# cloudflare/circl

Measured on AMD Instinct MI355X. Metric: ML-KEM-768 encapsulations/sec (whole node), batch=2^20, higher is better.
Workload: dtype i32; 1 GPU; ML-KEM-768 Encapsulate, distinct-key (one GPU-generated key per item), batch=1048576 per GPU, inputs resident in HBM (SURVEY 8d scope i; the PCIe-inclusive host-ABI rate, scope ii, is `value_host_abi`); key_pool=1048576, parallelism=batch split per device, no collectives, mode=encaps

## Files before the change

### circl_amd/csrc/api_mlkem.hip

```cpp
#include "host_common.h"
#include "keytable.h"
#include "mlkem_kernels.h"

using namespace circl::host;
using circl::KeyIdx;

namespace {

constexpr size_t kKemWsPerItem = 129;
size_t kem_scratch_bytes() { return 256 + max_resident_blocks() * 64 * 512; }
size_t kem_small_batch() {
    static const size_t v = [] {
        const char *e = getenv("CIRCL_HIP_KEM_SMALL");
        const int lg = e ? atoi(e) : 15;
        return lg <= 0 ? size_t(0) : size_t(1) << std::min(lg, 20);
    }();
    return v;
}
size_t kem_coop_batch() {
    static const size_t v = [] {
        const char *e = getenv("CIRCL_HIP_KEM_COOP");
        const int lg = e ? atoi(e) : 11;
        return lg <= 0 ? size_t(0) : size_t(1) << std::min(lg, 20);
    }();
// ... 51 lines not shown
struct KemWs {
    uint8_t *slot0, *slot1, *slot2, *slot3, *status_slot;
    unsigned *work;
    uint8_t *scratch;
    KemWs(void *ws, size_t n) {
        slot0 = static_cast<uint8_t *>(ws);
        slot1 = slot0 + 32 * n;
        slot2 = slot0 + 64 * n;
        slot3 = slot0 + 96 * n;
        status_slot = slot0 + 128 * n;
        work = reinterpret_cast<unsigned *>(slot0 + up256(kKemWsPerItem * n));
        scratch = slot0 + up256(kKemWsPerItem * n) + 256;
    }
};


template <int K, bool R3 = false>
int encaps_dev_impl(const uint8_t *ek, const uint8_t *m, uint8_t *ct, uint8_t *ss, uint8_t *status, size_t n,
                    void *ws, size_t ws_bytes, hipStream_t st) {
    using Gm = circl::mlkem::Geom<K>;
    using namespace circl::mlkem;
    if (n == 0) return CIRCL_HIP_OK;
    if (ws_bytes < kem_ws_min(n) || !aligned16(ws) || !aligned16(ek) || !aligned16(m) || !aligned16(ct) || !aligned16(ss))
        return CIRCL_HIP_EWORKSPACE;
    KemWs w(ws, n);
    uint8_t *r_ws = w.slot0, *m_ws = w.slot1;
    const unsigned hb = (unsigned)((n + 255) / 256);
    if (!R3 && n <= kem_chain_item_batch()) {
        ProfScope ps(CIRCL_HIP_KERNEL_MLKEM_ENCRYPT, st);
        hipLaunchKernelGGL((mlkem_encaps_chain_kernel<K, false>), dim3((unsigned)n), dim3(128), 0, st, ek, (size_t)Gm::EK, KeyIdx{},
                           (const int16_t *)nullptr, (const uint8_t *)nullptr, m, ct, ss, status, n);
        HIP_TRY(hipGetLastError());
        return CIRCL_HIP_OK;
    }
    if (!R3 && kem_small_route(n, ws_bytes)) {
        int16_t *key_rows = reinterpret_cast<int16_t *>(static_cast<uint8_t *>(ws) + kem_small_table_ofs(n));
        const int coop = kem_hash_form(n, kem_coop_batch());
        const unsigned nb_expand = (unsigned)((n + Gm::G - 1) / Gm::G), nb_hash = kem_hash_blocks(n, coop);
        static_assert(Gm::LDS_FIFO >= 108 * 8, "the cooperative hash's exchange area fits the FIFO area");
        const size_t want = kem_small_group(n);
        HIP_TRY(hipMemsetAsync(w.work, 0, 256, st));
        {
            ProfScope ps(CIRCL_HIP_KERNEL_MLKEM_HASH, st);
            hipLaunchKernelGGL(mlkem_small_pre_kernel<K>, dim3(nb_hash + nb_expand), dim3(64), Gm::LDS_FIFO, st, ek, m, ss, r_ws, key_rows, n, nb_hash, coop);
        }
        auto kern = mlkem_encrypt_kernel<K, ENCAPS, 0, true, KM_KEYED>;
        const unsigned eb = std::min<unsigned>((unsigned)((n + want - 1) / want), resident_blocks(kern, Gm::LDS_SHARED_TOTAL));
        ProfScope ps(CIRCL_HIP_KERNEL_MLKEM_ENCRYPT, st);
        hipLaunchKernelGGL(kern, dim3(eb), dim3(64), Gm::LDS_SHARED_TOTAL, st, ek, (size_t)Gm::EK, m, (const uint8_t *)r_ws, ct, ss, status,
                           (const uint8_t *)nullptr, (const uint8_t *)nullptr, w.scratch, w.work, n, KeyIdx{}, (const int16_t *)key_rows);
        HIP_TRY(hipGetLastError());
        return CIRCL_HIP_OK;
    }
    HIP_TRY(hipMemsetAsync(w.work, 0, 256, st));
    {
        ProfScope ps(CIRCL_HIP_KERNEL_MLKEM_HASH, st);
        if (R3) hipLaunchKernelGGL(kyber_r3_hash_kernel<K>, dim3(hb), dim3(256), 0, st, ek, m, ss, r_ws, m_ws, n);
        else hipLaunchKernelGGL(mlkem_hash_kernel<K>, dim3(hb), dim3(256), 0, st, ek, m, ss, r_ws, n);
    }
    {
        auto kern = mlkem_encrypt_kernel<K, R3 ? ENCAPS_LENIENT : ENCAPS, 0, true>;
        const unsigned eb = std::min<unsigned>((unsigned)((n + Gm::G - 1) / Gm::G), resident_blocks(kern, Gm::LDS_SCRATCH_TOTAL));
        ProfScope ps(CIRCL_HIP_KERNEL_MLKEM_ENCRYPT, st);
        hipLaunchKernelGGL(kern, dim3(eb), dim3(64), Gm::LDS_SCRATCH_TOTAL, st, ek, (size_t)Gm::EK, R3 ? (const uint8_t *)m_ws : m, (const uint8_t *)r_ws,
                           ct, ss, status, (const uint8_t *)nullptr, (const uint8_t *)nullptr, w.scratch, w.work, n, KeyIdx{},
                           (const int16_t *)nullptr);
    }
    if (R3) {
        ProfScope ps(CIRCL_HIP_KERNEL_MLKEM_HASH, st);
        hipLaunchKernelGGL(kyber_r3_finish_kernel<K>, dim3(hb), dim3(256), 0, st, (const uint8_t *)ct, ss, n);
    }
    HIP_TRY(hipGetLastError());
    return CIRCL_HIP_OK;
}

template <int K>
int encaps_shared_dev_impl(const uint8_t *ek, const uint8_t *m, uint8_t *ct, uint8_t *ss, uint8_t *status, size_t n, void *ws,
                           size_t ws_bytes, hipStream_t st) {
    using Gm = circl::mlkem::Geom<K>;
    using namespace circl::mlkem;
    if (n == 0) return CIRCL_HIP_OK;
    if (ws_bytes < kem_ws_min(n) || !aligned16(ws) || !aligned16(ek) || !aligned16(m) || !aligned16(ct) || !aligned16(ss))
        return CIRCL_HIP_EWORKSPACE;
    KemWs w(ws, n);
    uint8_t *r_ws = w.slot0, *h_ws = w.slot1;
    if (n <= kem_chain_item_batch()) {
        ProfScope ps(CIRCL_HIP_KERNEL_MLKEM_ENCRYPT, st);
        hipLaunchKernelGGL((mlkem_encaps_chain_kernel<K, false>), dim3((unsigned)n), dim3(128), 0, st, ek, (size_t)0, KeyIdx{},
                           (const int16_t *)nullptr, (const uint8_t *)nullptr, m, ct, ss, status, n);
        HIP_TRY(hipGetLastError());
        return CIRCL_HIP_OK;
    }
    HIP_TRY(hipMemsetAsync(w.work, 0, 256, st));
    if (n <= kem_small_shared_batch(false)) {
        int16_t *key_rows = reinterpret_cast<int16_t *>(static_cast<uint8_t *>(ws) + kem_small_table_ofs(n));
        static_assert(Gm::LDS_FIFO >= 108 * 8, "the cooperative hash's exchange area fits the FIFO area");
        {
            ProfScope ps(CIRCL_HIP_KERNEL_MLKEM_HASH, st);
            hipLaunchKernelGGL(mlkem_small_shared_pre_kernel<K>, dim3(1 + (unsigned)((n + 31) / 32)), dim3(64), Gm::LDS_FIFO, st, ek, m, ss, r_ws, key_rows, n);
        }
        auto kern = mlkem_encrypt_kernel<K, ENCAPS, 0, true, KM_KEYED>;
        const size_t want = kem_small_group(n);
        const unsigned eb = std::min<unsigned>((unsigned)((n + want - 1) / want), resident_blocks(kern, Gm::LDS_SHARED_TOTAL));
        ProfScope ps(CIRCL_HIP_KERNEL_MLKEM_ENCRYPT, st);
        hipLaunchKernelGGL(kern, dim3(eb), dim3(64), Gm::LDS_SHARED_TOTAL, st, ek, (size_t)0, m, (const uint8_t *)r_ws, ct, ss, status,
                           (const uint8_t *)nullptr, (const uint8_t *)nullptr, w.scratch, w.work, n, KeyIdx{}, (const int16_t *)key_rows);
        HIP_TRY(hipGetLastError());
        return CIRCL_HIP_OK;
    }
    {
        ProfScope ps(CIRCL_HIP_KERNEL_MLKEM_HASH, st);
        hipLaunchKernelGGL(mlkem_hek_kernel<K>, dim3(1), dim3(64), 0, st, ek, h_ws);
        hipLaunchKernelGGL(mlkem_g_shared_kernel, dim3((unsigned)((n + 255) / 256)), dim3(256), 0, st, (const uint8_t *)h_ws, m, ss,
                           r_ws, n, KeyIdx{});
    }
    {
        auto kern = mlkem_encrypt_kernel<K, ENCAPS, 0, true, KM_SHARED>;
        const unsigned eb = std::min<unsigned>((unsigned)((n + Gm::GS - 1) / Gm::GS), resident_blocks(kern, Gm::LDS_SHARED_TOTAL));
// ... 794 lines not shown
```

### circl_amd/csrc/mlkem_kernels.h

```cpp
#pragma once
#include "kyber_dev.h"

#ifndef CIRCL_KEM_RING_PRIO
#define CIRCL_KEM_RING_PRIO 1
#endif
#ifndef CIRCL_KEM_WAVES_PER_EU
#define CIRCL_KEM_WAVES_PER_EU 4
#endif

namespace circl {
namespace mlkem {

using kyber::Q;

template <int K> struct Params;
template <> struct Params<2> { static constexpr int ETA1 = 3, DU = 10, DV = 4; };
template <> struct Params<3> { static constexpr int ETA1 = 2, DU = 10, DV = 4; };
template <> struct Params<4> { static constexpr int ETA1 = 2, DU = 11, DV = 5; };

template <int K> struct Geom {
    using P = Params<K>;
    static constexpr int EK = 384 * K + 32;
    static constexpr int DK = 768 * K + 96;
    static constexpr int CT = 32 * (P::DU * K + P::DV);
    static constexpr int PAIRS = K * K;
    static constexpr int G = 64 / PAIRS;
    static constexpr int A_STREAMS = G * PAIRS;
    static constexpr int NOISE = 2 * K + 1;
    static constexpr int A_STRIDE = 520;
    static constexpr int NOISE_BYTES = 64 * P::ETA1;
    static constexpr int NOISE_STRIDE = NOISE_BYTES + 8;
    static constexpr int LDS_A = A_STREAMS * A_STRIDE;
    static constexpr int HALVES = K == 2 ? 2 : 1;
    static constexpr int GH = G / HALVES;
    static constexpr int LDS_NOISE = GH * NOISE * NOISE_STRIDE;
    static constexpr int LDS_XCH = 1024;
    static constexpr int LDS_TOTAL = LDS_A + LDS_NOISE + LDS_XCH;
    static constexpr int FIFO_STRIDE = 80;
    static constexpr int LDS_FIFO = 64 * FIFO_STRIDE;
    static constexpr int LDS_SCRATCH_TOTAL = (LDS_FIFO > LDS_NOISE + LDS_XCH) ? LDS_FIFO : LDS_NOISE + LDS_XCH;
    static constexpr int SCRATCH_BYTES = 64 * 512;
    static constexpr int GS = K == 2 ? 8 : 64 / NOISE;
    static constexpr int LDS_NOISE_SHARED = GS * NOISE * NOISE_STRIDE;
    static constexpr int LDS_SHARED_TOTAL = (LDS_FIFO > LDS_NOISE_SHARED + LDS_XCH) ? LDS_FIFO : LDS_NOISE_SHARED + LDS_XCH;
};


template <int FIRST, int COUNT> __device__ __forceinline__ void xor_words(KeccakState &s, const uint64_t *p) {
    detail::static_for<0, COUNT>([&](auto ic) {
        constexpr int i = decltype(ic)::v;
        const uint64_t w = p[i];
        s.lo[FIRST + i] ^= (uint32_t)w;
        s.hi[FIRST + i] ^= (uint32_t)(w >> 32);
    });
}

template <int NWORDS> __device__ __forceinline__ void sha3_256_words(KeccakState &s, const uint64_t *p) {
    constexpr int FULL = NWORDS / 17, REM = NWORDS % 17;
    keccak_zero(s);
#pragma unroll 1
    for (int b = 0; b < FULL; b++) {
        xor_words<0, 17>(s, p + 17 * b);
        keccak_f1600(s);
    }
    xor_words<0, REM>(s, p + 17 * FULL);
    s.lo[REM] ^= kDsSha3;
    s.hi[16] ^= 0x80000000u;
    keccak_f1600(s);
}

__device__ __forceinline__ void sha3_512_m_h(KeccakState &g, const uint64_t *m, const KeccakState &h) {
    keccak_zero(g);
    xor_words<0, 4>(g, m);
#pragma unroll
    for (int i = 0; i < 4; i++) { g.lo[4 + i] = h.lo[i]; g.hi[4 + i] = h.hi[i]; }
    g.lo[8] = kDsSha3;
    g.hi[8] = 0x80000000u;
    keccak_f1600(g);
}

template <int NWORDS, class Src> __device__ __forceinline__ void split_sponge17_src(SplitState &s, Src &&src, uint32_t ds, bool hi_lane) {
    constexpr int FULL = NWORDS / 17, REM = NWORDS % 17;
    uint32_t nx[17];
#pragma unroll
    for (int j = 0; j < 25; j++) s.w[j] = 0;
#pragma unroll
    for (int j = 0; j < 17; j++) nx[j] = (FULL > 0 || j < REM) ? src(j) : 0;
#pragma unroll 1
    for (int b = 0; b < FULL; b++) {
#pragma unroll
        for (int j = 0; j < 17; j++) s.w[j] ^= nx[j];
        const bool last = b + 1 == FULL;
#pragma unroll
// ... 13 lines not shown
                                              size_t item, bool live, int parity) {
    const bool hi_lane = parity != 0;
    const uint32_t *mw = reinterpret_cast<const uint32_t *>(m + item * 32) + parity;
    SplitState s;
#pragma unroll
    for (int j = 0; j < 4; j++) { s.w[j] = mw[2 * j]; s.w[4 + j] = h[j]; }
    s.w[8] = hi_lane ? 0x80000000u : kDsSha3;
#pragma unroll
    for (int j = 9; j < 25; j++) s.w[j] = 0;
    keccak_f1600_split(s, hi_lane);
    if (live) {
        uint32_t *kd = reinterpret_cast<uint32_t *>(ss + item * 32) + parity, *rd = reinterpret_cast<uint32_t *>(r_ws + item * 32) + parity;
#pragma unroll
        for (int j = 0; j < 4; j++) { kd[2 * j] = s.w[j]; rd[2 * j] = s.w[4 + j]; }
    }
}
template <int K>
__device__ __forceinline__ void mlkem_hash_split(const uint8_t *__restrict__ ek, const uint8_t *__restrict__ m, uint8_t *__restrict__ ss,
                                                 uint8_t *__restrict__ r_ws, size_t item, bool live, int parity) {
    using Gm = Geom<K>;
    SplitState s;
    split_sponge17<Gm::EK / 8>(s, reinterpret_cast<const uint32_t *>(ek + item * Gm::EK) + parity, kDsSha3, parity != 0);
    const uint32_t h[4] = {s.w[0], s.w[1], s.w[2], s.w[3]};
    mlkem_g_split(h, m, ss, r_ws, item, live, parity);
}

template <int FIRST, int COUNT> __device__ __forceinline__ void store_words(uint64_t *p, const KeccakState &s) {
    detail::static_for<0, COUNT>([&](auto ic) {
        constexpr int i = decltype(ic)::v;
        p[i] = ((uint64_t)s.hi[FIRST + i] << 32) | s.lo[FIRST + i];
    });
}

template <bool NW = false, class Src>
__device__ __forceinline__ void coop_sponge17(uint32_t &vlo, uint32_t &vhi, Src &&src, int nwords, uint32_t ds, const CoopLane &c, int j) {
    const int full = nwords / 17, rem = nwords % 17;
    vlo = vhi = 0;
    uint64_t next = j < 17 ? src(j) : 0;
#pragma unroll 1
    for (int b = 0; b < full; b++) {
        vlo ^= (uint32_t)next;
        vhi ^= (uint32_t)(next >> 32);
        next = (j < 17 && 17 * (b + 1) + j < nwords) ? src(17 * (b + 1) + j) : 0;
        keccak_f1600_coop2<NW>(vlo, vhi, c);
    }
    vlo ^= (uint32_t)next;
    vhi ^= (uint32_t)(next >> 32);
    if (j == rem) vlo ^= ds;
    if (j == 16) vhi ^= 0x80000000u;
    keccak_f1600_coop2<NW>(vlo, vhi, c);
}


template <int K>
__global__ void __launch_bounds__(256) mlkem_hash_kernel(const uint8_t *__restrict__ ek, const uint8_t *__restrict__ m,
                                                         uint8_t *__restrict__ ss, uint8_t *__restrict__ r_ws, size_t n) {
    using Gm = Geom<K>;
    size_t idx = (size_t)blockIdx.x * 256 + threadIdx.x;
    const bool live = idx < n;
    if (!live) idx = n - 1;
    KeccakState h, g;
    sha3_256_words<Gm::EK / 8>(h, reinterpret_cast<const uint64_t *>(ek + idx * Gm::EK));
    sha3_512_m_h(g, reinterpret_cast<const uint64_t *>(m + idx * 32), h);
    if (live) {
        store_words<0, 4>(reinterpret_cast<uint64_t *>(ss + idx * 32), g);
        store_words<4, 4>(reinterpret_cast<uint64_t *>(r_ws + idx * 32), g);
    }
}

template <int K>
__global__ void __launch_bounds__(64) mlkem_dk_check_kernel(const uint8_t *__restrict__ dk, uint8_t *__restrict__ key_status) {
    __shared__ uint64_t ws[100];
    const int lane = threadIdx.x, j = lane & 31;
    const CoopLane c = coop_lane(ws, lane);
    const uint64_t *ekw = reinterpret_cast<const uint64_t *>(dk + 384 * K);
    const uint64_t *stored = reinterpret_cast<const uint64_t *>(dk + 768 * K + 32);
    uint32_t vlo, vhi;
    coop_sponge17(vlo, vhi, [&](int k) { return ekw[k]; }, Geom<K>::EK / 8, kDsSha3, c, j);
    const bool mine = j >= 4 || ((((uint64_t)vhi << 32) | vlo) == stored[j & 3]);
    const unsigned long long bad = __ballot(!mine);
    if (lane == 0) *key_status = (bad & 0xfull) == 0 ? 0 : 2;
}


template <int K>
__global__ void __launch_bounds__(64) mlkem_hek_kernel(const uint8_t *__restrict__ ek, uint8_t *__restrict__ h_ws) {
    __shared__ uint64_t ws[100];
    const int lane = threadIdx.x, j = lane & 31;
    const CoopLane c = coop_lane(ws, lane);
    const uint64_t *ekw = reinterpret_cast<const uint64_t *>(ek);
    uint32_t vlo, vhi;
    coop_sponge17(vlo, vhi, [&](int k) { return ekw[k]; }, Geom<K>::EK / 8, kDsSha3, c, j);
    if (lane < 4) reinterpret_cast<uint64_t *>(h_ws)[lane] = ((uint64_t)vhi << 32) | vlo;
}

template <int K>
__global__ void __launch_bounds__(256) mlkem_hek_table_kernel(const uint8_t *__restrict__ keys, size_t stride, size_t ek_off,
                                                              uint8_t *__restrict__ h_out, uint8_t *__restrict__ key_status, int stored,
                                                              size_t nkeys) {
    size_t j = (size_t)blockIdx.x * 256 + threadIdx.x;
    const bool live = j < nkeys;
    if (!live) j = nkeys - 1;
    const uint8_t *ekp = keys + j * stride + ek_off;
    KeccakState h;
    sha3_256_words<Geom<K>::EK / 8>(h, reinterpret_cast<const uint64_t *>(ekp));
    if (!live) return;
    store_words<0, 4>(reinterpret_cast<uint64_t *>(h_out + j * 32), h);
    if (stored) {
        const uint64_t *st = reinterpret_cast<const uint64_t *>(ekp + Geom<K>::EK);
        bool ok = true;
#pragma unroll
        for (int i = 0; i < 4; i++) ok &= (((uint64_t)h.hi[i] << 32) | h.lo[i]) == st[i];
        key_status[j] = ok ? 0 : 2;
    }
}
static __global__ void __launch_bounds__(256) mlkem_g_shared_kernel(const uint8_t *__restrict__ h_ws, const uint8_t *__restrict__ m,
                                                             uint8_t *__restrict__ ss, uint8_t *__restrict__ r_ws, size_t n,
                                                             const KeyIdx key_idx) {
    const size_t idx = (size_t)blockIdx.x * 256 + threadIdx.x;
    if (idx >= n) return;
// ... 137 lines not shown
            fifo[cnt & (SLOTS - 1)] = (int16_t)v;
            count_accept(cnt, v);
            if constexpr (c % 8 == 7) {
                cnt = min(cnt, 256);
                if (cnt - flushed >= 8) {
                    const uint4 d = *reinterpret_cast<const uint4 *>(fifo + (flushed & (SLOTS - 1)));
                    *reinterpret_cast<uint4 *>(row + flushed) = d;
                    flushed += 8;
                }
                if constexpr (TAIL) live = __any(flushed < 256);
            }
        }
    });
}

template <int K, bool TRANSPOSED, int GA = Geom<K>::G, bool XY_ARG = false>
__device__ __forceinline__ void sample_matrix_scratch(uint8_t *lds_fifo, int16_t *rows, const uint8_t *__restrict__ rho,
                                                      size_t rho_stride, size_t item0, size_t n, int lane, const uint8_t *__restrict__ xy = nullptr) {
    using Gm = Geom<K>;
    const bool on = XY_ARG ? item0 + lane < n : lane < GA * Gm::PAIRS;
    const int g = XY_ARG ? lane : on ? lane / Gm::PAIRS : 0, p = on ? lane % Gm::PAIRS : 0;
    const int i = p / K, j = p % K;
    size_t item = item0 + g;
    if (item >= n) item = n - 1;
    KeccakState s;
    keccak_zero(s);
    xor_words<0, 4>(s, reinterpret_cast<const uint64_t *>(rho + item * rho_stride));
    if constexpr (XY_ARG) s.lo[4] = (uint32_t)xy[2 * item] | ((uint32_t)xy[2 * item + 1] << 8) | (kDsShake << 16);
    else s.lo[4] = (TRANSPOSED ? (uint32_t)i | ((uint32_t)j << 8) : (uint32_t)j | ((uint32_t)i << 8)) | (kDsShake << 16);
    s.hi[20] = 0x80000000u;
    int16_t *fifo = reinterpret_cast<int16_t *>(lds_fifo + lane * Gm::FIFO_STRIDE);
    int16_t *row = rows + lane * 256;
    int cnt = on ? 0 : 256, flushed = cnt;
#pragma unroll 1
    for (int blk = 0; blk < 3; blk++) {
        keccak_f1600(s);
        if (on) parse_shake128_block_fifo<false>(s, fifo, row, cnt, flushed);
    }
#pragma unroll 1
    while (__any(flushed < 256)) {
        keccak_f1600(s);
        parse_shake128_block_fifo<true>(s, fifo, row, cnt, flushed);
    }
}

template <bool ETA2> __device__ __forceinline__ void store_prf_words(uint32_t *out, const KeccakState &s) {
    detail::static_for<0, 16>([&](auto ic) {
        constexpr int w = decltype(ic)::v;
        out[2 * w] = ETA2 ? kyber::cbd2_bias8_word(s.lo[w]) : s.lo[w];
        out[2 * w + 1] = ETA2 ? kyber::cbd2_bias8_word(s.hi[w]) : s.hi[w];
    });
}

template <int K, bool TRANSPOSED, int NOISE, int ETA1_COUNT>
__device__ __forceinline__ void sample_matrix_and_prf(uint8_t *lds_fifo, uint8_t *lds_noise, uint8_t *lds_mini, int16_t *rows,
                                                      const uint8_t *__restrict__ rho, size_t rho_stride,
                                                      const uint8_t *__restrict__ seed, size_t seed_stride, size_t item0, size_t n,
                                                      int lane) {
    using Gm = Geom<K>;
    constexpr int STREAMS = Gm::G * NOISE;
    constexpr int LAST_BASE = ((STREAMS - 1) / 64) * 64, USED_LAST = STREAMS - LAST_BASE, FREE = 64 - USED_LAST;
    constexpr int MAX_HITCH = FREE < 15 ? FREE : 15;
    constexpr bool CAN_HITCH = Params<K>::ETA1 == 2 && MAX_HITCH > 0;
    constexpr int STASH = 240;
    static_assert(15 * STASH <= Gm::LDS_FIFO, "stash fits in the FIFO area");

    KeccakState s;
    int cnt, flushed;
    int16_t *fifo = reinterpret_cast<int16_t *>(lds_fifo + lane * Gm::FIFO_STRIDE);
    {
        const bool on = lane < Gm::A_STREAMS;
        const int g = on ? lane / Gm::PAIRS : 0, p = on ? lane % Gm::PAIRS : 0;
        const int i = p / K, j = p % K;
        size_t item = item0 + g;
        if (item >= n) item = n - 1;
        keccak_zero(s);
        xor_words<0, 4>(s, reinterpret_cast<const uint64_t *>(rho + item * rho_stride));
        s.lo[4] = (TRANSPOSED ? (uint32_t)i | ((uint32_t)j << 8) : (uint32_t)j | ((uint32_t)i << 8)) | (kDsShake << 16);
        s.hi[20] = 0x80000000u;
        int16_t *row = rows + lane * 256;
        cnt = on ? 0 : 256;
        flushed = cnt;
#pragma unroll 1
        for (int blk = 0; blk < 3; blk++) {
            keccak_f1600(s);
            if (on) parse_shake128_block_fifo<false>(s, fifo, row, cnt, flushed);
        }
        const unsigned long long smask0 = __ballot(flushed < 256);
        if (!CAN_HITCH || __popcll(smask0) > MAX_HITCH) {
#pragma unroll 1
            while (__any(flushed < 256)) {
                keccak_f1600(s);
                parse_shake128_block_fifo<true>(s, fifo, row, cnt, flushed);
            }
        }
    }
    const unsigned long long smask = __ballot(flushed < 256);
    const int nstr = __popcll(smask);
    if (nstr > 0) {
        const bool mine = (smask >> lane) & 1;
        uint4 pend = make_uint4(0, 0, 0, 0);
        if (mine) pend = *reinterpret_cast<const uint4 *>(fifo + (flushed & 31));
        __syncthreads();
        if (mine) {
            uint32_t *st = reinterpret_cast<uint32_t *>(lds_fifo + __popcll(smask & ((1ull << lane) - 1)) * STASH);
#pragma unroll
            for (int w = 0; w < 25; w++) { st[2 * w] = s.lo[w]; st[2 * w + 1] = s.hi[w]; }
            st[50] = (uint32_t)cnt; st[51] = (uint32_t)flushed; st[52] = (uint32_t)lane;
            st[53] = pend.x; st[54] = pend.y; st[55] = pend.z; st[56] = pend.w;
        }
    }
    __syncthreads();

#pragma unroll 1
    for (int base = 0; base < STREAMS; base += 64) {
        const int sidx = base + lane;
        const bool on = sidx < STREAMS;
        const int g = on ? sidx / NOISE : 0, nonce = on ? sidx % NOISE : 0;
        size_t item = item0 + g;
        if (item >= n) item = n - 1;
        keccak_zero(s);
        xor_words<0, 4>(s, reinterpret_cast<const uint64_t *>(seed + item * seed_stride));
        s.lo[4] = (uint32_t)nonce | (kDsShake << 8);
        s.hi[16] = 0x80000000u;
        const bool adopt_pass = CAN_HITCH && nstr > 0 && base == LAST_BASE;
        const int tk = lane - USED_LAST;
        const bool target = adopt_pass && tk >= 0 && tk < nstr;
        int tcnt = 256, tflushed = 256, tsrc = 0;
        uint4 pend = make_uint4(0, 0, 0, 0);
        if (target) {
            const uint32_t *st = reinterpret_cast<const uint32_t *>(lds_fifo + tk * STASH);
#pragma unroll
            for (int w = 0; w < 25; w++) { s.lo[w] = st[2 * w]; s.hi[w] = st[2 * w + 1]; }
            tcnt = (int)st[50]; tflushed = (int)st[51]; tsrc = (int)st[52];
            pend = make_uint4(st[53], st[54], st[55], st[56]);
        }
        keccak_f1600(s);
        uint32_t *out = reinterpret_cast<uint32_t *>(lds_noise + (on ? sidx : 0) * Gm::NOISE_STRIDE);
        if constexpr (Params<K>::ETA1 == 2) {
            if (on) store_prf_words<true>(out, s);
        } else {
            if (on && nonce < ETA1_COUNT) store_prf_words<false>(out, s);
            if (on && nonce >= ETA1_COUNT) store_prf_words<true>(out, s);
        }
        if constexpr (Params<K>::ETA1 == 3) {
            if (on && nonce < ETA1_COUNT) { out[32] = s.lo[16]; out[33] = s.hi[16]; }
            if (__any(on && nonce < ETA1_COUNT)) {
                keccak_f1600(s);
                if (on && nonce < ETA1_COUNT) {
                    detail::static_for<0, 7>([&](auto ic) {
                        constexpr int w = decltype(ic)::v;
                        out[34 + 2 * w] = s.lo[w];
                        out[35 + 2 * w] = s.hi[w];
                    });
                }
            }
        }
        if (adopt_pass) {
            int16_t *tf = reinterpret_cast<int16_t *>(lds_mini + (target ? tk : 15) * 32);
            int16_t *trow = rows + tsrc * 256;
            if (target) *reinterpret_cast<uint4 *>(tf + (tflushed & 15)) = pend;
            parse_shake128_block_fifo<true, 16>(s, tf, trow, tcnt, tflushed);
#pragma unroll 1
            while (__any(tflushed < 256)) {
                keccak_f1600(s);
                parse_shake128_block_fifo<true, 16>(s, tf, trow, tcnt, tflushed);
            }
        }
    }
}

struct AFromLds {
    const uint8_t *base;
    int stride;
    __device__ __forceinline__ void load(uint32_t &a01, uint32_t &a23, int stream, int lane) const {
        const uint2 w = *reinterpret_cast<const uint2 *>(base + stream * stride + 8 * lane);
        a01 = w.x; a23 = w.y;
    }
};
struct AFromScratch {
    const int16_t *rows;
    __device__ __forceinline__ void load(uint32_t &a01, uint32_t &a23, int stream, int lane) const {
        const uint64_t w = __hip_atomic_load(reinterpret_cast<const uint64_t *>(rows + stream * 256 + 4 * lane), __ATOMIC_RELAXED,
                                             __HIP_MEMORY_SCOPE_AGENT);
        a01 = (uint32_t)w; a23 = (uint32_t)(w >> 32);
    }
};
struct AFromCache {
    const int16_t *rows;
    __device__ __forceinline__ void load(uint32_t &a01, uint32_t &a23, int stream, int lane) const {
        const uint2 w = *reinterpret_cast<const uint2 *>(rows + stream * 256 + 4 * lane);
        a01 = w.x; a23 = w.y;
    }
};
__device__ __forceinline__ void rows_acquire() {
    __builtin_amdgcn_fence(__ATOMIC_RELEASE, "workgroup");
    __syncthreads();
    __builtin_amdgcn_fence(__ATOMIC_ACQUIRE, "agent");
}


template <int K, int NOISE, int ETA1_COUNT, int GCOUNT = Geom<K>::G>
__device__ __forceinline__ void prf_streams(uint8_t *lds_noise, const uint8_t *__restrict__ seed, size_t seed_stride,
                                            size_t item0, size_t n, int lane, int g0 = 0) {
    using Gm = Geom<K>;
    constexpr int STREAMS = GCOUNT * NOISE;
#pragma unroll 1
    for (int base = 0; base < STREAMS; base += 64) {
        const int sidx = base + lane;
        const bool on = sidx < STREAMS;
        const int g = g0 + (on ? sidx / NOISE : 0), nonce = on ? sidx % NOISE : 0;
        size_t item = item0 + g;
        if (item >= n) item = n - 1;
        KeccakState s;
        keccak_zero(s);
        xor_words<0, 4>(s, reinterpret_cast<const uint64_t *>(seed + item * seed_stride));
        s.lo[4] = (uint32_t)nonce | (kDsShake << 8);
        s.hi[16] = 0x80000000u;
        keccak_f1600(s);
        uint32_t *out = reinterpret_cast<uint32_t *>(lds_noise + (on ? sidx : 0) * Gm::NOISE_STRIDE);
        if constexpr (Params<K>::ETA1 == 2) {
            if (on) store_prf_words<true>(out, s);
// ... 173 lines not shown
}

template <int D> __device__ __forceinline__ unsigned get_bits(const uint8_t *p, int n) {
    const int bit = n * D, b = bit >> 3, sh = bit & 7;
    unsigned w = p[b];
    if (sh + D > 8) w |= (unsigned)p[b + 1] << 8;
    if (sh + D > 16) w |= (unsigned)p[b + 2] << 16;
    return (w >> sh) & ((1u << D) - 1);
}

__device__ __forceinline__ size_t next_group(unsigned *work, int lane, bool first, size_t ngroups) {
    if (first) return (size_t)blockIdx.x;
    if (work == nullptr || (size_t)gridDim.x >= ngroups) return ngroups;
    unsigned t = 0;
    if (lane == 0) t = atomicAdd(work, 1u);
    return (size_t)gridDim.x + (size_t)(unsigned)__builtin_amdgcn_readfirstlane((int)t);
}


enum EncryptMode { ENCAPS = 0, REENCRYPT = 1, ENCAPS_LENIENT = 2 };

enum KeyMode { KM_ITEM = 0, KM_SHARED = 1, KM_KEYED = 2 };
template <int K, int MODE, int ABLATE_ARG = 0, bool SCRATCH = true, int KM = KM_ITEM>
__global__ void __launch_bounds__(64, SCRATCH ? CIRCL_KEM_WAVES_PER_EU : 1) mlkem_encrypt_kernel(const uint8_t *__restrict__ ek, size_t ek_stride,
                                                          const uint8_t *__restrict__ m, const uint8_t *__restrict__ r_ws,
                                                          uint8_t *__restrict__ ct, uint8_t *__restrict__ ss,
                                                          uint8_t *__restrict__ status, const uint8_t *__restrict__ kbar_ws,
                                                          const uint8_t *__restrict__ ssrej_ws, uint8_t *__restrict__ scratch, unsigned *__restrict__ work, size_t n,
                                                          const KeyIdx key_idx, const int16_t *__restrict__ key_rows) {
    using Gm = Geom<K>;
    using P = Params<K>;
    constexpr int ABLATE = ABLATE_ARG & 7;
    constexpr bool CLK = (ABLATE_ARG & 8) != 0;
    uint64_t clk[4] = {0, 0, 0, 0}, tprev = 0;
    auto lap = [&](int slot) {
        if constexpr (CLK) {
            const uint64_t t = __builtin_readcyclecounter();
            clk[slot] += t - tprev;
            tprev = t;
        }
    };
    if constexpr (CLK) tprev = __builtin_readcyclecounter();
    extern __shared__ __attribute__((aligned(16))) uint8_t smem[];
    uint8_t *lds_a = smem;
    uint8_t *lds_noise = SCRATCH ? smem : smem + Gm::LDS_A;
    constexpr bool SHARED = KM != KM_ITEM;
    static_assert(!SHARED || (SCRATCH && (MODE == ENCAPS || MODE == REENCRYPT) && ABLATE == 0), "shared-key / key-table mode");
    uint8_t *xch = lds_noise + (SHARED ? Gm::LDS_NOISE_SHARED : Gm::LDS_NOISE);
    int16_t *rows = KM == KM_KEYED ? nullptr : reinterpret_cast<int16_t *>(scratch + (size_t)blockIdx.x * Gm::SCRATCH_BYTES);
    const int lane = threadIdx.x;
    constexpr int GI = SHARED ? Gm::GS : Gm::G;
    const unsigned gi = (SHARED && (size_t)gridDim.x * GI >= n) ? (unsigned)((n + gridDim.x - 1) / gridDim.x) : (unsigned)GI;
    const size_t ngroups = (n + gi - 1) / gi;
    if constexpr (KM == KM_SHARED) {
        sample_matrix_scratch<K, true, 1>(lds_a, rows, ek + 384 * K, 0, 0, 1, lane);
        __threadfence_block();
        __syncthreads();
    }

#pragma unroll 1
  for (size_t grp = next_group(work, lane, true, ngroups); grp < ngroups; grp = next_group(work, lane, false, ngroups)) {
    const size_t item0 = grp * gi;
    lap(0);
    if constexpr (CIRCL_KEM_RING_PRIO != 0) __builtin_amdgcn_s_setprio(0);
    if constexpr (SHARED) {
        __syncthreads();
        if (gi * Gm::NOISE <= 32) prf_streams_split<K, Gm::NOISE, K>(lds_noise, r_ws, 32, item0, n, lane, (int)gi);
        else prf_streams<K, Gm::NOISE, K, Gm::GS>(lds_noise, r_ws, 32, item0, n, lane);
        __syncthreads();
    } else if constexpr (SCRATCH && ABLATE == 0 && Gm::HALVES == 1) {
        __syncthreads();
        sample_matrix_and_prf<K, true, Gm::NOISE, K>(lds_a, lds_noise, xch, rows, ek + 384 * K, ek_stride,
                                                     r_ws, 32, item0, n, lane);
        __threadfence_block();
        __syncthreads();
    } else {
        if (!(ABLATE & 1)) {
            if constexpr (SCRATCH) {
                __syncthreads();
                sample_matrix_scratch<K, true>(lds_a, rows, ek + 384 * K, ek_stride, item0, n, lane);
                __threadfence_block();
            } else {
                sample_matrix<K, true>(lds_a, ek + 384 * K, ek_stride, item0, n, lane);
            }
        }
        __syncthreads();
        if constexpr (Gm::HALVES == 1) {
            if (!(ABLATE & 2)) prf_streams<K, Gm::NOISE, K>(lds_noise, r_ws, 32, item0, n, lane);
            __syncthreads();
        }
    }

    int lane_ring = lane;
    asm volatile("" : "+v"(lane_ring));
    if constexpr (CIRCL_KEM_RING_PRIO != 0) __builtin_amdgcn_s_setprio(CIRCL_KEM_RING_PRIO);
    lap(1);
    const kyber::LaneZetas z = kyber::load_lane_zetas(lane_ring);
#pragma unroll 1
    for (int g = 0; g < ((ABLATE & 4) ? 0 : (int)gi); g++) {
        const size_t item = item0 + g;
        if (item >= n) break;
        if constexpr (Gm::HALVES > 1 && !SHARED) {
            if (g % Gm::GH == 0) {
                __syncthreads();
                if (!(ABLATE & 2)) prf_streams<K, Gm::NOISE, K, Gm::GH>(lds_noise, r_ws, 32, item0, n, lane, g);
                __syncthreads();
            }
        }
        const size_t kq = KM == KM_KEYED ? (key_idx ? (size_t)key_idx[item] : (ek_stride ? item : size_t(0))) : item;
        const uint8_t *ekp = ek + kq * ek_stride;
        const int16_t *krows = KM == KM_KEYED ? key_rows + kq * (size_t)(K * K * 256) : nullptr;
        const uint8_t *noise = lds_noise + (SHARED ? g : g % Gm::GH) * Gm::NOISE * Gm::NOISE_STRIDE;

        int th[K][4];
        bool bad = false;
#pragma unroll
        for (int j = 0; j < K; j++) {
            unpack12_l4(th[j], ekp + 384 * j, lane);
#pragma unroll
            for (int r = 0; r < 4; r++) {
                if (MODE == ENCAPS) bad |= th[j][r] >= Q;
                else th[j][r] = kyber::csubq(th[j][r]);
            }
        }
        const bool reject = MODE == ENCAPS ? __any(bad) : false;

// ... 24 lines not shown
                else AFromLds{lds_a, Gm::A_STRIDE}.load(a01, a23, (g * K + i) * K + j, lane);
                kyber::mulhat_acc_packed(acc, a01, a23, rop[j]);
            }
            kyber::mulhat_finish(acc);
            kyber::invntt<kyber::NEG_R32, CIRCL_KEM_RING_XCH>(acc, z, xch, lane);
            const uint8_t *e1 = noise + (K + i) * Gm::NOISE_STRIDE;
            unsigned cv[4];
#pragma unroll
            for (int r = 0; r < 4; r++)
                cv[r] = kyber::compress_coeff<P::DU>(acc[r] + cbd_coeff<2>(e1, kyber::idx_l1(lane, r)));
            uint32_t *stage = reinterpret_cast<uint32_t *>(xch);
            stage_bits_l1<P::DU>(stage, cv, lane);
            if (MODE == REENCRYPT) differs |= ref.differs(stage, lane);
            else store_staged<P::DU>(dst, stage, lane, reject);
        }
        {
            uint32_t *dst = reinterpret_cast<uint32_t *>(ctp + 32 * P::DU * K);
            RefWords<P::DV> ref;
            if (MODE == REENCRYPT) ref.load(dst, lane);
            int acc[4] = {0, 0, 0, 0};
#pragma unroll
            for (int j = 0; j < K; j++) kyber::mulhat_acc_packed(acc, kyber::pack16(th[j][0], th[j][1]), kyber::pack16(th[j][2], th[j][3]), rop[j]);
            kyber::mulhat_finish(acc);
            kyber::invntt<kyber::NEG_R32, CIRCL_KEM_RING_XCH>(acc, z, xch, lane);
            const uint8_t *e2 = noise + 2 * K * Gm::NOISE_STRIDE;
            const uint8_t *mp = m + item * 32;
            unsigned cv[4];
#pragma unroll
            for (int r = 0; r < 4; r++) {
                const int nidx = kyber::idx_l1(lane, r);
                const int mbit = (mp[nidx >> 3] >> (nidx & 7)) & 1;
                cv[r] = kyber::compress_coeff<P::DV>(acc[r] + cbd_coeff<2>(e2, nidx) + (-mbit & ((Q + 1) / 2)));
            }
            uint32_t *stage = reinterpret_cast<uint32_t *>(xch);
            stage_bits_l1<P::DV>(stage, cv, lane);
            if (MODE == REENCRYPT) differs |= ref.differs(stage, lane);
            else store_staged<P::DV>(dst, stage, lane, reject);
        }
        if (MODE == ENCAPS) {
            if (lane == 0) status[item] = reject ? 1 : 0;
            if (reject && lane < 8) reinterpret_cast<uint32_t *>(ss + item * 32)[lane] = 0;
        } else if (MODE == REENCRYPT) {
            const bool mismatch = __any(differs);
            const bool dead = status[item] != 0;
            if (lane < 8) {
                const uint32_t kb = reinterpret_cast<const uint32_t *>(kbar_ws + item * 32)[lane];
                const uint32_t rj = reinterpret_cast<const uint32_t *>(ssrej_ws + item * 32)[lane];
                reinterpret_cast<uint32_t *>(ss + item * 32)[lane] = dead ? 0u : (mismatch ? rj : kb);
            }
        }
        if constexpr (CLK) clk[3]++;
    }
    lap(2);
  }
    if constexpr (CLK) {
        lap(0);
        if (lane == 0) {
            uint64_t *prof = reinterpret_cast<uint64_t *>(const_cast<int16_t *>(key_rows)) + (size_t)blockIdx.x * 4;
#pragma unroll
            for (int q = 0; q < 4; q++) prof[q] = clk[q];
        }
    }
}

template <int K>
__global__ void __launch_bounds__(64, CIRCL_KEM_WAVES_PER_EU) mlkem_expand_keys_kernel(const uint8_t *__restrict__ keys, size_t stride, size_t rho_off,
                                                                                      int16_t *__restrict__ key_rows, size_t nkeys) {
    using Gm = Geom<K>;
    extern __shared__ __attribute__((aligned(16))) uint8_t smem[];
    const size_t e0 = (size_t)blockIdx.x * Gm::G;
    sample_matrix_scratch<K, true>(smem, key_rows + e0 * (size_t)(K * K * 256), keys + rho_off, stride, e0, nkeys, threadIdx.x);
}

template <int K>
__device__ __forceinline__ void mlkem_hash_coop2(const uint8_t *__restrict__ ek, const uint8_t *__restrict__ m, uint8_t *__restrict__ ss,
                                                 uint8_t *__restrict__ r_ws, size_t item0, size_t n, uint64_t *ws, int lane) {
    using Gm = Geom<K>;
    constexpr int NW = Gm::EK / 8, FULL = NW / 17, REM = NW % 17;
    const CoopLane c = coop_lane(ws, lane);
    uint64_t *hx = ws + 100;
    const int half = lane >> 5, j = lane & 31;
    size_t item = item0 + half;
    const bool live = item < n;
    if (!live) item = n - 1;
    const uint64_t *ekw = reinterpret_cast<const uint64_t *>(ek + item * Gm::EK);
    uint32_t vlo = 0, vhi = 0;
    uint64_t next = j < 17 ? ekw[j] : 0;
#pragma unroll 1
    for (int b = 0; b < FULL; b++) {
        vlo ^= (uint32_t)next;
        vhi ^= (uint32_t)(next >> 32);
        next = (j < 17 && 17 * (b + 1) + j < NW) ? ekw[17 * (b + 1) + j] : 0;
        keccak_f1600_coop2(vlo, vhi, c);
    }
    vlo ^= (uint32_t)next;
    vhi ^= (uint32_t)(next >> 32);
    if (j == REM) vlo ^= kDsSha3;
    if (j == 16) vhi ^= 0x80000000u;
    keccak_f1600_coop2(vlo, vhi, c);
    __syncthreads();
    if (j < 4) hx[4 * half + j] = ((uint64_t)vhi << 32) | vlo;
    __syncthreads();
    uint64_t g = 0;
    if (j < 4) g = reinterpret_cast<const uint64_t *>(m + item * 32)[j];
    else if (j < 8) g = hx[4 * half + j - 4];
    else if (j == 8) g = 0x8000000000000000ull | kDsSha3;
    vlo = (uint32_t)g;
// ... 907 lines not shown
```

Baseline: 142.6 million encaps/s.

## Fuse the SHA3-512 G hash into idle lanes of the encrypt kernel's PRF pass

For ML-KEM with ETA1=2, the hash kernel now computes only H(ek) for most groups and writes it to a workspace. The G = SHA3-512(m||H(ek)) permutation for the next work-stealing group runs on spare lanes of the last PRF Keccak pass inside the encrypt kernel. The resulting r seed is held in LDS, so the next group reads it from there instead of from global r_ws. The hash kernel also zeroes the work counter itself, dropping a separate memset. This is meant to remove a global round trip and a separate Keccak permutation per item. In exchange it adds LDS, prefetches tickets one group ahead, takes hitch lanes away from the PRF pass, and adds control complexity.

Measured after the change: 143.0 million encaps/s (median of 6 runs). Within noise of the previous version (+0.2%).

```diff
diff --git a/circl_amd/csrc/api_mlkem.hip b/circl_amd/csrc/api_mlkem.hip
--- a/circl_amd/csrc/api_mlkem.hip
+++ b/circl_amd/csrc/api_mlkem.hip
@@ -127,18 +127,23 @@
         HIP_TRY(hipGetLastError());
         return CIRCL_HIP_OK;
     }
-    HIP_TRY(hipMemsetAsync(w.work, 0, 256, st));
-    {
-        ProfScope ps(CIRCL_HIP_KERNEL_MLKEM_HASH, st);
+    auto kern = mlkem_encrypt_kernel<K, R3 ? ENCAPS_LENIENT : ENCAPS, 0, true>;
+    const size_t ngroups = (n + Gm::G - 1) / Gm::G;
+    const unsigned eb = std::min<unsigned>((unsigned)ngroups, resident_blocks(kern, Gm::LDS_SCRATCH_TOTAL));
+    constexpr bool G_RIDE = CIRCL_KEM_G_RIDE != 0 && !R3 && Params<K>::ETA1 == 2;
+    uint8_t *hek_ws = G_RIDE ? w.slot1 : nullptr;
+    if (!G_RIDE) HIP_TRY(hipMemsetAsync(w.work, 0, 256, st));
+    {
+        ProfScope ps(CIRCL_HIP_KERNEL_MLKEM_HASH, st);
+        const GRideRange rr = g_ride_range(ngroups, eb);
         if (R3) hipLaunchKernelGGL(kyber_r3_hash_kernel<K>, dim3(hb), dim3(256), 0, st, ek, m, ss, r_ws, m_ws, n);
-        else hipLaunchKernelGGL(mlkem_hash_kernel<K>, dim3(hb), dim3(256), 0, st, ek, m, ss, r_ws, n);
-    }
-    {
-        auto kern = mlkem_encrypt_kernel<K, R3 ? ENCAPS_LENIENT : ENCAPS, 0, true>;
-        const unsigned eb = std::min<unsigned>((unsigned)((n + Gm::G - 1) / Gm::G), resident_blocks(kern, Gm::LDS_SCRATCH_TOTAL));
+        else hipLaunchKernelGGL(mlkem_hash_kernel<K>, dim3(hb), dim3(256), 0, st, ek, m, ss, r_ws, n, hek_ws, G_RIDE ? w.work : (unsigned *)nullptr,
+                                rr.lo * Gm::G, rr.hi * Gm::G);
+    }
+    {
         ProfScope ps(CIRCL_HIP_KERNEL_MLKEM_ENCRYPT, st);
         hipLaunchKernelGGL(kern, dim3(eb), dim3(64), Gm::LDS_SCRATCH_TOTAL, st, ek, (size_t)Gm::EK, R3 ? (const uint8_t *)m_ws : m, (const uint8_t *)r_ws,
-                           ct, ss, status, (const uint8_t *)nullptr, (const uint8_t *)nullptr, w.scratch, w.work, n, KeyIdx{},
+                           ct, ss, status, (const uint8_t *)hek_ws, (const uint8_t *)nullptr, w.scratch, w.work, n, KeyIdx{},
                            (const int16_t *)nullptr);
     }
     if (R3) {
diff --git a/circl_amd/csrc/mlkem_kernels.h b/circl_amd/csrc/mlkem_kernels.h
--- a/circl_amd/csrc/mlkem_kernels.h
+++ b/circl_amd/csrc/mlkem_kernels.h
@@ -1,4 +1,6 @@
 #pragma once
+#include <type_traits>
+
 #include "kyber_dev.h"
 
 #ifndef CIRCL_KEM_RING_PRIO
@@ -38,7 +40,8 @@
     static constexpr int LDS_TOTAL = LDS_A + LDS_NOISE + LDS_XCH;
     static constexpr int FIFO_STRIDE = 80;
     static constexpr int LDS_FIFO = 64 * FIFO_STRIDE;
-    static constexpr int LDS_SCRATCH_TOTAL = (LDS_FIFO > LDS_NOISE + LDS_XCH) ? LDS_FIFO : LDS_NOISE + LDS_XCH;
+    static constexpr int LDS_RIDE = P::ETA1 == 2 ? G * 32 + 16 : 0;
+    static constexpr int LDS_SCRATCH_TOTAL = ((LDS_FIFO > LDS_NOISE + LDS_XCH) ? LDS_FIFO : LDS_NOISE + LDS_XCH) + LDS_RIDE;
     static constexpr int SCRATCH_BYTES = 64 * 512;
     static constexpr int GS = K == 2 ? 8 : 64 / NOISE;
     static constexpr int LDS_NOISE_SHARED = GS * NOISE * NOISE_STRIDE;
@@ -158,20 +161,35 @@
 }
 
 
+#ifndef CIRCL_KEM_G_RIDE
+#define CIRCL_KEM_G_RIDE 1
+#endif
+constexpr size_t G_RIDE_TAIL = 2;
+struct GRideRange { size_t lo, hi; };
+__host__ __device__ inline GRideRange g_ride_range(size_t ngroups, size_t grid) {
+    return GRideRange{grid, ngroups > (1 + G_RIDE_TAIL) * grid ? ngroups - G_RIDE_TAIL * grid : grid};
+}
+
 template <int K>
 __global__ void __launch_bounds__(256) mlkem_hash_kernel(const uint8_t *__restrict__ ek, const uint8_t *__restrict__ m,
-                                                         uint8_t *__restrict__ ss, uint8_t *__restrict__ r_ws, size_t n) {
+                                                         uint8_t *__restrict__ ss, uint8_t *__restrict__ r_ws, size_t n,
+                                                         uint8_t *__restrict__ hek_ws, unsigned *__restrict__ work, size_t ride_lo, size_t ride_hi) {
     using Gm = Geom<K>;
     size_t idx = (size_t)blockIdx.x * 256 + threadIdx.x;
+    if (work != nullptr && idx < 64) work[idx] = 0;
     const bool live = idx < n;
     if (!live) idx = n - 1;
     KeccakState h, g;
     sha3_256_words<Gm::EK / 8>(h, reinterpret_cast<const uint64_t *>(ek + idx * Gm::EK));
-    sha3_512_m_h(g, reinterpret_cast<const uint64_t *>(m + idx * 32), h);
-    if (live) {
-        store_words<0, 4>(reinterpret_cast<uint64_t *>(ss + idx * 32), g);
-        store_words<4, 4>(reinterpret_cast<uint64_t *>(r_ws + idx * 32), g);
-    }
+    const bool rides = hek_ws != nullptr && idx >= ride_lo && idx < ride_hi;
+    if (__any(live && !rides)) {
+        sha3_512_m_h(g, reinterpret_cast<const uint64_t *>(m + idx * 32), h);
+        if (live && !rides) {
+            store_words<0, 4>(reinterpret_cast<uint64_t *>(ss + idx * 32), g);
+            store_words<4, 4>(reinterpret_cast<uint64_t *>(r_ws + idx * 32), g);
+        }
+    }
+    if (live && rides) store_words<0, 4>(reinterpret_cast<uint64_t *>(hek_ws + idx * 32), h);
 }
 
 template <int K>
@@ -415,15 +433,38 @@
     });
 }
 
-template <int K, bool TRANSPOSED, int NOISE, int ETA1_COUNT>
+__device__ __forceinline__ size_t next_group(unsigned *work, int lane, bool first, size_t ngroups);
+struct NoGRide { static constexpr int LANES = 0; };
+template <int K> struct GRide {
+    static constexpr int LANES = Geom<K>::G;
+    const uint8_t *m;
+    uint8_t *ss;
+    uint8_t *lds_r;
+    unsigned *work;
+    size_t ngroups, grp;
+    struct Parked {
+        unsigned hi;
+        unsigned nxt;
+        const uint8_t *hek;
+    };
+    __device__ __forceinline__ Parked *parked() const { return reinterpret_cast<Parked *>(lds_r + LANES * 32); }
+    __device__ __forceinline__ unsigned hi() const { return (unsigned)__builtin_amdgcn_readfirstlane((int)parked()->hi); }
+    __device__ __forceinline__ unsigned nxt() const { return (unsigned)__builtin_amdgcn_readfirstlane((int)parked()->nxt); }
+    static constexpr unsigned NO_TICKET = ~0u;
+    static __device__ __forceinline__ bool rides(size_t g, unsigned hi) { return g >= gridDim.x && g < hi; }
+};
+template <int K, bool TRANSPOSED, int NOISE, int ETA1_COUNT, class Ride>
 __device__ __forceinline__ void sample_matrix_and_prf(uint8_t *lds_fifo, uint8_t *lds_noise, uint8_t *lds_mini, int16_t *rows,
                                                       const uint8_t *__restrict__ rho, size_t rho_stride,
                                                       const uint8_t *__restrict__ seed, size_t seed_stride, size_t item0, size_t n,
-                                                      int lane) {
+                                                      int lane, Ride &ride) {
     using Gm = Geom<K>;
     constexpr int STREAMS = Gm::G * NOISE;
     constexpr int LAST_BASE = ((STREAMS - 1) / 64) * 64, USED_LAST = STREAMS - LAST_BASE, FREE = 64 - USED_LAST;
-    constexpr int MAX_HITCH = FREE < 15 ? FREE : 15;
+    constexpr int RIDERS = Ride::LANES;
+    constexpr bool RIDE = RIDERS > 0;
+    static_assert(!RIDE || (Params<K>::ETA1 == 2 && RIDERS <= FREE), "G rides on idle lanes of a one-permutation PRF pass");
+    constexpr int MAX_HITCH = FREE - RIDERS < 15 ? FREE - RIDERS : 15;
     constexpr bool CAN_HITCH = Params<K>::ETA1 == 2 && MAX_HITCH > 0;
     constexpr int STASH = 240;
     static_assert(15 * STASH <= Gm::LDS_FIFO, "stash fits in the FIFO area");
@@ -475,6 +516,19 @@
     }
     __syncthreads();
 
+    bool seed_lds = false, ride_pass = false;
+    unsigned ride_nxt = 0;
+    if constexpr (RIDE) {
+        const unsigned hi = ride.hi();
+        seed_lds = Ride::rides(ride.grp, hi);
+        if (ride.grp < hi) {
+            ride_nxt = (unsigned)next_group(ride.work, lane, false, ride.ngroups);
+            ride_pass = Ride::rides(ride_nxt, hi);
+        } else {
+            ride_nxt = Ride::NO_TICKET;
+        }
+        if (lane == 0) ride.parked()->nxt = ride_nxt;
+    }
 #pragma unroll 1
     for (int base = 0; base < STREAMS; base += 64) {
         const int sidx = base + lane;
@@ -483,11 +537,31 @@
         size_t item = item0 + g;
         if (item >= n) item = n - 1;
         keccak_zero(s);
-        xor_words<0, 4>(s, reinterpret_cast<const uint64_t *>(seed + item * seed_stride));
+        if constexpr (RIDE) {
+            if (seed_lds) xor_words<0, 4>(s, reinterpret_cast<const uint64_t *>(ride.lds_r + g * 32));
+            else xor_words<0, 4>(s, reinterpret_cast<const uint64_t *>(seed + item * seed_stride));
+        } else {
+            xor_words<0, 4>(s, reinterpret_cast<const uint64_t *>(seed + item * seed_stride));
+        }
         s.lo[4] = (uint32_t)nonce | (kDsShake << 8);
         s.hi[16] = 0x80000000u;
+        if constexpr (RIDE) {
+            const int rk = lane - USED_LAST;
+            if (ride_pass && base == LAST_BASE && rk >= 0 && rk < RIDERS) {
+                const size_t ritem = (size_t)ride_nxt * RIDERS + rk;
+                const uint64_t *mw = reinterpret_cast<const uint64_t *>(ride.m + ritem * 32), *hw = reinterpret_cast<const uint64_t *>(ride.parked()->hek + ritem * 32);
+#pragma unroll
+                for (int w = 0; w < 4; w++) {
+                    s.lo[w] = (uint32_t)mw[w]; s.hi[w] = (uint32_t)(mw[w] >> 32);
+                    s.lo[4 + w] = (uint32_t)hw[w]; s.hi[4 + w] = (uint32_t)(hw[w] >> 32);
+                }
+                s.lo[8] = kDsSha3;
+                s.hi[8] = 0x80000000u;
+                s.hi[16] = 0;
+            }
+        }
         const bool adopt_pass = CAN_HITCH && nstr > 0 && base == LAST_BASE;
-        const int tk = lane - USED_LAST;
+        const int tk = lane - USED_LAST - RIDERS;
         const bool target = adopt_pass && tk >= 0 && tk < nstr;
         int tcnt = 256, tflushed = 256, tsrc = 0;
         uint4 pend = make_uint4(0, 0, 0, 0);
@@ -499,6 +573,13 @@
             pend = make_uint4(st[53], st[54], st[55], st[56]);
         }
         keccak_f1600(s);
+        if constexpr (RIDE) {
+            const int rk = lane - USED_LAST;
+            if (ride_pass && base == LAST_BASE && rk >= 0 && rk < RIDERS) {
+                store_words<0, 4>(reinterpret_cast<uint64_t *>(ride.ss + ((size_t)ride_nxt * RIDERS + rk) * 32), s);
+                store_words<4, 4>(reinterpret_cast<uint64_t *>(ride.lds_r + rk * 32), s);
+            }
+        }
         uint32_t *out = reinterpret_cast<uint32_t *>(lds_noise + (on ? sidx : 0) * Gm::NOISE_STRIDE);
         if constexpr (Params<K>::ETA1 == 2) {
             if (on) store_prf_words<true>(out, s);
@@ -531,6 +612,14 @@
             }
         }
     }
+}
+template <int K, bool TRANSPOSED, int NOISE, int ETA1_COUNT>
+__device__ __forceinline__ void sample_matrix_and_prf(uint8_t *lds_fifo, uint8_t *lds_noise, uint8_t *lds_mini, int16_t *rows,
+                                                      const uint8_t *__restrict__ rho, size_t rho_stride,
+                                                      const uint8_t *__restrict__ seed, size_t seed_stride, size_t item0, size_t n,
+                                                      int lane) {
+    NoGRide none;
+    sample_matrix_and_prf<K, TRANSPOSED, NOISE, ETA1_COUNT>(lds_fifo, lds_noise, lds_mini, rows, rho, rho_stride, seed, seed_stride, item0, n, lane, none);
 }
 
 struct AFromLds {
@@ -810,6 +899,15 @@
     constexpr int GI = SHARED ? Gm::GS : Gm::G;
     const unsigned gi = (SHARED && (size_t)gridDim.x * GI >= n) ? (unsigned)((n + gridDim.x - 1) / gridDim.x) : (unsigned)GI;
     const size_t ngroups = (n + gi - 1) / gi;
+    constexpr bool G_RIDE = CIRCL_KEM_G_RIDE != 0 && MODE == ENCAPS && KM == KM_ITEM && SCRATCH && ABLATE == 0 && Gm::HALVES == 1;
+    using Ride = std::conditional_t<G_RIDE, GRide<K>, NoGRide>;
+    Ride ride;
+    if constexpr (G_RIDE) {
+        const GRideRange rr = g_ride_range(ngroups, gridDim.x);
+        ride.m = m; ride.ss = ss; ride.lds_r = xch + Gm::LDS_XCH; ride.work = work; ride.ngroups = ngroups;
+        static_assert(sizeof(typename Ride::Parked) == 16 && Gm::LDS_RIDE == Gm::G * 32 + 16, "GRide's LDS");
+        if (lane == 0) *ride.parked() = typename Ride::Parked{kbar_ws != nullptr && rr.lo < rr.hi ? (unsigned)rr.hi : 0u, 0u, kbar_ws};
+    }
     if constexpr (KM == KM_SHARED) {
         sample_matrix_scratch<K, true, 1>(lds_a, rows, ek + 384 * K, 0, 0, 1, lane);
         __threadfence_block();
@@ -817,7 +915,7 @@
     }
 
 #pragma unroll 1
-  for (size_t grp = next_group(work, lane, true, ngroups); grp < ngroups; grp = next_group(work, lane, false, ngroups)) {
+  for (size_t grp = next_group(work, lane, true, ngroups); grp < ngroups;) {
     const size_t item0 = grp * gi;
     lap(0);
     if constexpr (CIRCL_KEM_RING_PRIO != 0) __builtin_amdgcn_s_setprio(0);
@@ -828,8 +926,9 @@
         __syncthreads();
     } else if constexpr (SCRATCH && ABLATE == 0 && Gm::HALVES == 1) {
         __syncthreads();
+        if constexpr (G_RIDE) ride.grp = grp;
         sample_matrix_and_prf<K, true, Gm::NOISE, K>(lds_a, lds_noise, xch, rows, ek + 384 * K, ek_stride,
-                                                     r_ws, 32, item0, n, lane);
+                                                     r_ws, 32, item0, n, lane, ride);
         __threadfence_block();
         __syncthreads();
     } else {
@@ -960,7 +1059,16 @@
         if constexpr (CLK) clk[3]++;
     }
     lap(2);
+    if constexpr (G_RIDE) {
+        const unsigned nx = ride.nxt();
+        grp = nx != Ride::NO_TICKET ? (size_t)nx : next_group(work, lane, false, ngroups);
+    } else {
+        grp = next_group(work, lane, false, ngroups);
+    }
   }
+    if constexpr (G_RIDE) {
+        if (lane < Gm::G * 8) reinterpret_cast<uint32_t *>(ride.lds_r)[lane] = 0;
+    }
     if constexpr (CLK) {
         lap(0);
         if (lane == 0) {
```
